# Guoxs/DODT

Hardware: AMD Instinct MI355X
Metric: frame-pairs/sec (whole node) KITTI-shape tau=2 (higher is better)
Workload: dtype f32

## Files before the change

dodt_amd/_lib.py:

```python
import ctypes as C
import os

_HERE = os.path.dirname(os.path.abspath(__file__))
LIB_PATH = os.environ.get('DODT_HIP_LIB') or os.path.join(_HERE, 'lib', 'libdodt_hip.so')

OK, ERR_INVALID, ERR_HIP, ERR_UNSUPPORTED = 0, 1, 2, 3
PTS_VELO_XYZI, PTS_CAM_3XN = 0, 1
EXTRACTOR_VGG_PYR = 0
EXTRACTOR_VGG = 1
EXTRACTOR_SHARED_GPU = 0x100
EXTRACTOR_BF16 = 0x200
EXTRACTOR_SPLIT = 0x400
FC_RELU = 1
FC_BF16 = 2
CONFLICT_RAISE, CONFLICT_NEXT_BEST = 0, 1


class DodtError(RuntimeError):
    pass


class BevParams(C.Structure):
    _fields_ = [
        ('point_format', C.c_int32),
# ... 83 lines not shown
    'dodt_bev_slices': (_i, [_vp, _vp, _i, C.POINTER(BevParams), _pf, _vp]),
    'dodt_bev_status': (_i, [_vp, C.POINTER(_i)]),
    'dodt_bev_support_mask': (_i, [C.POINTER(BevParams), _i, _vp, _i, _i]),
    'dodt_anchor_filter': (_i, [_vp, _vp, _i, _i, _pi32, _i, _i, _pi32, _pi32]),
    'dodt_project_anchors_f64': (_i, [_vp, _vp, _pi32, _i, _pi32,
                                      C.POINTER(_d), C.POINTER(_d), _d, _d,
                                      _pf, _pf, _pf]),
    'dodt_project_anchors_f32': (_i, [_vp, _pf, _i, _pi32, C.POINTER(_f),
                                      C.POINTER(_f), _f, _f, _pf, _pf, _pf]),
    'dodt_img_preprocess': (_i, [_vp, _vp, _i, _i, _i, _i, _i,
                                 C.POINTER(_f), _pf]),
    'dodt_conv_mode': (_i, []),
    'dodt_extractor_create': (_i, [_vp, _i, _i, _i, _i, _i, _i,
                                   C.POINTER(_vp)]),
    'dodt_extractor_destroy': (_i, [_vp]),
    'dodt_extractor_set_layer': (_i, [_vp, C.c_char_p, _vp, _i, _i, _i, _i,
                                      _vp, _vp, _vp]),
    'dodt_extractor_input': (_i, [_vp, C.POINTER(_vp), C.POINTER(C.c_longlong)]),
    'dodt_extractor_forward': (_i, [_vp, _pf, _pf, _pf]),
    'dodt_extractor_forward_padded': (_i, [_vp, _pf, _pf, _pf]),
    'dodt_extractor_set_input': (_i, [_vp, _pf]),
    'dodt_extractor_set_input_support': (_i, [_vp, _vp, _i, _i, C.POINTER(C.c_longlong)]),
    'dodt_extractor_set_frame_tables': (_i, [_vp, _i, C.POINTER(_i)]),
    'dodt_extractor_frame_items': (_i, [_vp, C.POINTER(_i), _i]),
    'dodt_extractor_frame_split': (_i, [_vp, C.POINTER(_i), C.POINTER(_i), _i]),
    'dodt_extractor_store_bytes': (C.c_longlong, [_vp]),
    'dodt_frame_tables_host': (_i, [_vp, _i, _i, _i, _i, _i, _i, _vp, _i, _vp, _vp, C.POINTER(_i)]),
    'dodt_frame_restore_host': (_i, [_vp, _i, _i, _i, _i, _i, _i, _i, _i, _i, _vp, _vp, _vp, _vp]),
    'dodt_frame_lists_host': (_i, [_vp, _i, _i, _i, _i, _i, _i, _vp, _i, _vp, _vp, C.POINTER(_i), _vp, C.POINTER(_i)]),
    'dodt_extractor_read_activation': (_i, [_vp, C.c_char_p, _vp,
                                            C.POINTER(_i), C.POINTER(_i),
                                            C.POINTER(_i)]),
    'dodt_extractor_output_shape': (_i, [_vp, C.POINTER(_i), C.POINTER(_i), C.POINTER(_i)]),
    'dodt_extractor_first_layers_folded': (_i, [_vp]),
    'dodt_extractor_flops': (_d, [_vp]),
    'dodt_extractor_mfma_flops': (_d, [_vp]),
    'dodt_extractor_bytes': (_d, [_vp]),
    'dodt_extractor_layer_count': (_i, [_vp]),
    'dodt_conv_variant_count': (_i, []),
    'dodt_conv_variant_info': (_i, [_i, C.POINTER(ConvVariant)]),
    'dodt_conv_plan_host': (_i, [_i, _i, _i, _i, _i, _i, _i, C.POINTER(ConvLayerPlan), _i, C.POINTER(_i)]),
    'dodt_extractor_layer_plan': (_i, [_vp, C.POINTER(ConvLayerPlan), _i, C.POINTER(_i)]),
    'dodt_extractor_forward_timed': (_i, [_vp, _pf, _pf, _pf, C.POINTER(LayerInfo), _i]),
    'dodt_crop_and_resize': (_i, [_vp, _pf, _i, _i, _i, _pf, _i, _pi32, _i, _i,
                                  _pf]),
    'dodt_crop_and_resize_strided': (_i, [_vp, _pf, _i, _i, _i, _pf, _i, _pi32, _i, _i, _pf,
# ... 90 lines not shown
```

dodt_amd/csrc/conv.hip:

```cpp
#include <cmath>
#include <cstring>

#include <algorithm>
#include <utility>

#include "conv_variants.h"
#include "extractor.h"

using namespace dodt;

const std::vector<KernelVariant>& dodt::variants() {
    static const std::vector<KernelVariant> v = {
        InstSmall<32, 16, 6>::variant(),
        InstSmall<16, 12, 4>::variant(),
        InstSmall<16, 16, 6>::variant(),
        InstSmall<16, 16, 4>::variant(),
        Inst<32, 16, 4, 1, 32, false>::variant(),
        Inst<16, 16, 4, 1, 32, false>::variant(),
        Inst<16, 8, 4, 1, 64, false>::variant(),
        Inst<16, 12, 4, 1, 32, false>::variant(),
        Inst<8, 8, 4, 1, 32, false>::variant(),
        Inst<8, 8, 4, 1, 64, false>::variant(),
        Inst<8, 4, 2, 2, 128, false>::variant(),
        Inst<8, 4, 4, 1, 64, false>::variant(),
// ... 232 lines not shown
        *reinterpret_cast<f32x4*>(out + (size_t)pix * (LPP * 4) + l * 4) = v;
        if (bneck_out) {
            const f32x4 w = *reinterpret_cast<const f32x4*>(bneck_w + l * 4);
            dot = ((v[0] * w[0] + v[1] * w[1]) + v[2] * w[2]) + v[3] * w[3];
        }
    }
    if (bneck_out) {
#pragma unroll
        for (int m = 1; m < LPP; m <<= 1) dot += __shfl_xor(dot, m, 64);
        if (ok && l == 0) bneck_out[pix] = fmaxf(dot * bneck_scale + bneck_shift, 0.0f);
    }
}

int find_layer(dodt_extractor* ex, const char* name) {
    for (size_t i = 0; i < ex->layers.size(); ++i)
        if (ex->layers[i].name == name) return (int)i;
    return -1;
}

void report_launch(const dodt_extractor* ex, const Layer& l, const KernelVariant& v, const ConvArgs& a, int grid_x) {
    if (a.debug & 32) {
        int h[74];
        (void)hipStreamSynchronize(ex->ctx->stream);
        (void)hipMemcpy(h, ex->d_counters + 64 + 32, sizeof(h), hipMemcpyDeviceToHost);
        fprintf(stderr, "[dodt] %s step stamps (cycles): copies | transform | MFMAs | wait copies | barrier | step\n",
                l.name.c_str());
        for (int k = 0; k < 12; ++k)
            fprintf(stderr, "[dodt]   step %2d: %6d %6d %6d %6d %6d   next-top %6d\n", k, h[k * 6 + 1] - h[k * 6],
                    h[k * 6 + 2] - h[k * 6 + 1], h[k * 6 + 3] - h[k * 6 + 2], h[k * 6 + 4] - h[k * 6 + 3],
                    h[k * 6 + 5] - h[k * 6 + 4], k < 11 ? h[(k + 1) * 6] - h[k * 6] : 0);
        if (h[73] != h[72])
            fprintf(stderr, "[dodt]   steps 0..11: %d stamp ticks in %d ticks of the 100 MHz clock (%.0f MHz)\n",
                    h[66] - h[0], h[73] - h[72], 100.0 * (h[66] - h[0]) / (h[73] - h[72]));
    }
    if ((a.debug & 128) && v.dma) {
        std::vector<int> h(4 * grid_x);
        (void)hipStreamSynchronize(ex->ctx->stream);
        (void)hipMemcpy(h.data(), ex->d_counters + 64 + 256, h.size() * sizeof(int), hipMemcpyDeviceToHost);
        int t0 = h[0], s_max = h[0], f_max = h[1], e_min = h[2], e_max = h[2], items[8] = {};
        double first_sum = 0, run_sum = 0;
        for (int b = 0; b < (int)grid_x; ++b) {
            t0 = std::min(t0, h[4 * b]); s_max = std::max(s_max, h[4 * b]);
            f_max = std::max(f_max, h[4 * b + 1]);
            e_min = std::min(e_min, h[4 * b + 2]); e_max = std::max(e_max, h[4 * b + 2]);
            items[std::min(h[4 * b + 3], 7)]++;
            first_sum += (h[4 * b + 1] - h[4 * b]) / 100.0;
            run_sum += (h[4 * b + 2] - h[4 * b + 1]) / 100.0 / std::max(h[4 * b + 3], 1);
        }
        fprintf(stderr, "[dodt] %-16s %4d wgs, %5d items x %d chunks: last start +%.2f us, last first-step +%.2f, first end +%.2f, "
                "last end +%.2f; mean start->first step %.2f us, mean per item %.2f us; wgs by item count:",
                l.name.c_str(), (int)grid_x, a.n_items, a.Cin / 16, (s_max - t0) / 100.0, (f_max - t0) / 100.0,
                (e_min - t0) / 100.0, (e_max - t0) / 100.0, first_sum / grid_x, run_sum / grid_x);
        for (int k = 0; k < 8; ++k) if (items[k]) fprintf(stderr, " %d:%d", k, items[k]);
        int mt[2] = {0, 0};
        (void)hipMemcpy(mt, ex->d_counters + 64 + 250, sizeof(mt), hipMemcpyDeviceToHost);
        fprintf(stderr, "; shader clock of workgroup 1: %.2f GHz\n", (mt[1] - mt[0]) / ((h[4 + 2] - h[4 + 0]) * 10.0));
    }
    if (a.debug & 8) {
        unsigned long long h[2] = {0, 0};
        (void)hipStreamSynchronize(ex->ctx->stream);
        (void)hipMemcpy(h, ex->d_counters + 96, sizeof(h), hipMemcpyDeviceToHost);
        if (h[1])
            fprintf(stderr, "[dodt] %-16s wg0: %.1f us, shader clock %.3f GHz\n", l.name.c_str(),
                    h[1] / 100.0, (double)h[0] / h[1] * 0.1);
    }
}

int launch_grid(const KernelVariant& v, int n_items, int num_cus) {
    static const int bpc_env = getenv("DODT_CONV_BPC") ? atoi(getenv("DODT_CONV_BPC")) : 0;
    static const int small_bpc = getenv("DODT_CONV_SMALL_BPC") ? atoi(getenv("DODT_CONV_SMALL_BPC")) : 3;
    const int vb = v.small_cin ? small_bpc : v.blocks_per_cu;
    const int bpc = (bpc_env > 0 && bpc_env < vb) ? bpc_env : vb;
    return std::min(n_items, num_cus * bpc);
}

int run_launch(const dodt_extractor* ex, const Pass& p, const Layer& l, int which,
               float* override_out, int out_y0, int out_h, float* bneck_out, int pool_dst, const Layer* folded = nullptr) {
    const Launch& ln = which ? l.tail : l.main;
    const size_t li = &l - ex->layers.data();
    const ItemTable& t = p.table[li][which];
    const KernelVariant& v = variants()[folded ? ex->first2_variant : ln.variant];
    const int src_id = folded ? folded->src : l.src;
    const Buffer& src = ex->buf[src_id];
    const Buffer& dst = ex->buf[l.dst];
    ConvArgs a;
    a.in = p.map[src_id];
    a.out = override_out ? override_out : p.map[l.dst];
    a.w = ln.d_w ? ln.d_w : l.main.d_w;
    a.scale = l.d_scale;
    a.shift = l.d_shift;
    a.H = l.H;
    a.W = l.W;
    a.Cin = l.Cin;
    a.Cout = l.Cout;
    a.in_ld = src.C;
    a.in_coff = folded ? folded->src_coff : l.src_coff;
    a.out_ld = dst.C;
    a.out_coff = l.dst_coff;
    a.in_frame_stride = (long long)src.frame_floats();
    a.out_frame_stride = override_out ? (long long)out_h * dst.W * dst.C : (long long)dst.frame_floats();
    a.tiles_x = dodt::ceil_div(l.W, v.TW);
    a.tiles_y = dodt::ceil_div(l.H, v.TH);
    a.relu = 1;
    a.out_y0 = out_y0;
    a.out_nhwc = override_out ? 1 : 0;
    {
        static const int dbg = getenv("DODT_CONV_DEBUG") ? atoi(getenv("DODT_CONV_DEBUG")) : 0;
        a.debug = dbg;
        static const char* stamp_layer = getenv("DODT_CONV_STAMP_LAYER");
        if (stamp_layer && l.name == stamp_layer) a.debug |= 32;
    }
    a.counter = ex->d_counters + 2 * li + which;
    a.counter_base = ex->d_counters + 64;
    a.xcd_counters = variant_xcd_queue(v) ? ex->d_counters + 2048 + 128 * li : nullptr;
    a.items = v.small_cin && t.dense && t.n == a.tiles_x * a.tiles_y * p.frames ? nullptr : t.items;
    a.n_items = t.n;
    if (a.n_items == 0) return DODT_OK;
    a.n_items_dev = t.n_dev;
    a.in_part_stride = (long long)src.frame_floats() * p.frames;
    a.out_part_stride = (long long)dst.frame_floats() * p.frames;
    a.pool_part_stride = pool_dst >= 0 ? (long long)ex->buf[pool_dst].frame_floats() * p.frames : 0;
    a.pool_out = pool_dst >= 0 ? p.map[pool_dst] : nullptr;
    a.pool_frame_stride = pool_dst >= 0 ? (long long)ex->buf[pool_dst].frame_floats() : 0;
    a.bneck_w = bneck_out ? ex->d_bneck_w : nullptr;
    a.bneck_out = bneck_out;
    a.bneck_scale = ex->bneck_scale;
    a.bneck_shift = ex->bneck_shift;
    a.bneck_frame_stride = (long long)out_h * dst.W;
    a.zeros = ex->d_zeros;
    a.first_w = folded ? folded->d_first_w : nullptr;
    a.first_scale = folded ? folded->d_scale : nullptr;
    a.first_shift = folded ? folded->d_shift : nullptr;
    const int grid_x = launch_grid(v, a.n_items, ex->num_cus);
    dim3 grid(grid_x, 1);
    v.launch(a, grid, ex->ctx->stream);
    DODT_LAUNCH_CHECK();
    if (a.debug & (32 | 128 | 8)) report_launch(ex, l, v, a, grid_x);
    return DODT_OK;
}

bool variant_can_pool(const KernelVariant& v) {
    if (v.wino) return true;
    const int rows_per_mt = 32 / v.TW, mt = v.MTB / v.WM;
    return !v.deconv && !v.small_cin && (rows_per_mt >= 2 || mt % 2 == 0) && v.TH % 2 == 0;
}

bool layer_can_pool(const Layer& l) {
    return variant_can_pool(variants()[l.main.variant]) &&
           (l.tail.n_items == 0 || variant_can_pool(variants()[l.tail.variant]));
}

int run_layer(const dodt_extractor* ex, const Pass& p, const Layer& l, float* override_out, int out_y0, int out_h,
              float* bneck_out = nullptr, int pool_dst = -1, const Layer* folded = nullptr) {
    if (p.timed && folded) {
        DODT_HIP_CHECK(hipEventRecord(folded->ev0, ex->ctx->stream));
        DODT_HIP_CHECK(hipEventRecord(folded->ev1, ex->ctx->stream));
// ... 109 lines not shown
    const Buffer& s = ex->buf[src];
    const Buffer& d = ex->buf[dst];
    const int planes = d.C / 8;
    const long long total = (long long)p.frames * planes * d.H * d.W * 2;
    hipLaunchKernelGGL(maxpool2x2_kernel, dim3((unsigned)((total + 255) / 256)), dim3(256), 0,
                       ex->ctx->stream, p.map[src], s.H, s.W, planes, (long long)s.frame_floats(),
                       p.map[dst], p.frames);
    DODT_LAUNCH_CHECK();
    return DODT_OK;
}

int forward(dodt_extractor* ex, const float* d_in, const float* d_x0, float* d_feat_out, float* d_bottleneck_out,
            bool timed);

}

int dodt::fused_pool_buffer(const Layer& l) {
    static const bool no_fuse = getenv("DODT_CONV_NO_POOL_FUSE") != nullptr;
    return no_fuse || !layer_can_pool(l) ? -1 : l.pool;
}

bool dodt::bneck_fused(const Layer& last) {
    return variants()[last.main.variant].BN == 32 && (last.tail.n_items == 0 || variants()[last.tail.variant].BN == 32);
}

int dodt::run_layers(const dodt_extractor* ex, const Pass& p, float* d_feat_out, float* d_bottleneck_out) {
    hipStream_t s = ex->ctx->stream;
    int rc;
    const std::vector<Layer>& ls = ex->layers;
    if (ex->bf16)
        for (int id : {CONV1_2, CONV2_2, CONV3_3})
            DODT_REQUIRE(fused_pool_buffer(ls[id]) >= 0, "bf16 extractor: layer %s cannot pool in its epilogue",
                         ls[id].name.c_str());
    for (int id = ex->first2_variant >= 0 ? CONV1_2 : CONV1_1; id <= CONV4_3; ++id) {
        const Layer& l = ls[id];
        const Layer* folded = id == CONV1_2 && ex->first2_variant >= 0 ? &ls[CONV1_1] : nullptr;
        const int pool_dst = folded ? l.pool : fused_pool_buffer(l);
        if ((rc = run_layer(ex, p, l, nullptr, 0, 0, nullptr, pool_dst, folded))) return rc;
        if (l.pool >= 0 && pool_dst < 0 && (rc = run_pool(ex, p, l.dst, l.pool))) return rc;
    }
    if (ex->kind == DODT_EXTRACTOR_VGG) {
        const Buffer& c4 = ex->buf[C4C];
        const long long n_pix = (long long)p.frames * ex->out_h * ex->out_w;
        constexpr int kLpp = 64;
        hipLaunchKernelGGL(upsample_bilinear_cb8_kernel<kLpp>,
                           dim3((unsigned)((n_pix * kLpp + 255) / 256)), dim3(256), 0, s, p.map[C4C],
// ... 92 lines not shown
    for (Layer& l : plan.layers) {
        plan_layer(l, batch, num_cus, !shared_gpu, l.main.h_items, l.tail.h_items);
        l.main.n_items = (int)l.main.h_items.size();
        l.tail.n_items = (int)l.tail.h_items.size();
    }
    {
        static const bool first2 = !(getenv("DODT_CONV_BF16_FIRST2") && atoi(getenv("DODT_CONV_BF16_FIRST2")) == 0);
        const Layer& c11 = plan.layers[CONV1_1];
        const Layer& c12 = plan.layers[CONV1_2];
        const auto& vs = variants();
        if (first2 && bf16 && plan.parts == 1 && vs[c12.variant].stream_nch == 2 && c12.tail.n_items == 0 &&
            c11.Cout == 32 && c11.src_coff == 0 && (W * c11.Cin * 4) % 16 == 0 &&
            variant_can_pool(vs[c12.variant]))
            for (size_t i = 0; i < vs.size() && plan.first2_variant < 0; ++i)
                if (vs[i].first2 == c11.Cin && vs[i].TH == vs[c12.variant].TH && vs[i].TW == vs[c12.variant].TW &&
                    vs[i].lds_bytes <= (getenv("DODT_CONV_BF16_STREAM_LDS") ? atoi(getenv("DODT_CONV_BF16_STREAM_LDS")) * 1024 : 1 << 30))
                    plan.first2_variant = (int)i;
    }
    return DODT_OK;
}

namespace {

void report_layer(const std::vector<Layer>& layers, int first2_variant, int num_cus, size_t i, dodt_conv_layer_plan* o) {
    const Layer& l = layers[i];
    const bool folding = first2_variant >= 0;
    memset(o, 0, sizeof(*o));
    snprintf(o->name, sizeof(o->name), "%s", l.name.c_str());
    o->h = l.H; o->w = l.W; o->cin = l.Cin; o->cout = l.Cout;
    o->variant[0] = l.main.variant;
    o->variant[1] = l.tail.n_items > 0 ? l.tail.variant : -1;
    o->items[0] = l.main.n_items;
    o->items[1] = l.tail.n_items;
    if (folding && i == CONV1_1) {
        o->variant[0] = -1;
        o->items[0] = 0;
        o->folded = 1;
    }
    if (folding && i == CONV1_2) o->variant[0] = first2_variant;
    for (int j = 0; j < 2; ++j)
        o->grid[j] = o->variant[j] >= 0 ? launch_grid(variants()[o->variant[j]], o->items[j], num_cus) : 0;
    o->pool_fused = l.pool >= 0 && ((folding && i == CONV1_2) || fused_pool_buffer(l) >= 0);
    o->bneck_fused = i == FUSION1 && bneck_fused(l);
}

int report_plan(const std::vector<Layer>& layers, int first2_variant, int num_cus, dodt_conv_layer_plan* out, int n_out,
                int* n_layers) {
    if (n_layers) *n_layers = (int)layers.size();
    if (!out) return DODT_OK;
    DODT_REQUIRE(n_out >= (int)layers.size(), "conv plan: room for %d layers, the net has %d", n_out, (int)layers.size());
    for (size_t i = 0; i < layers.size(); ++i) report_layer(layers, first2_variant, num_cus, i, out + i);
    return DODT_OK;
}

}

extern "C" {

int dodt_conv_plan_host(int kind, int in_h, int in_w, int in_c, int pad_top, int batch, int num_cus,
                        dodt_conv_layer_plan* out, int n_out, int* n_layers) {
    ConvPlan plan;
    const int rc = plan_convs(kind, in_h, in_w, in_c, pad_top, batch, num_cus, plan);
    return rc ? rc : report_plan(plan.layers, plan.first2_variant, num_cus, out, n_out, n_layers);
}

int dodt_extractor_layer_plan(const dodt_extractor* ex, dodt_conv_layer_plan* out, int n_out, int* n_layers) {
    DODT_REQUIRE(ex, "dodt_extractor_layer_plan: extractor is NULL");
    return report_plan(ex->layers, ex->first2_variant, ex->num_cus, out, n_out, n_layers);
}

int dodt_conv_variant_count(void) { return (int)variants().size(); }

int dodt_conv_variant_info(int i, dodt_conv_variant* out) {
    DODT_REQUIRE(out && i >= 0 && i < (int)variants().size(), "dodt_conv_variant_info: bad argument");
    const KernelVariant& v = variants()[i];
    memset(out, 0, sizeof(*out));
    out->tw = v.TW; out->th = v.TH; out->bn = v.BN; out->ck = v.CK;
    out->blocks_per_cu = v.blocks_per_cu;
    out->flags = (v.deconv ? DODT_VARIANT_DECONV : 0) | (v.small_cin ? DODT_VARIANT_SMALL_CIN : 0) |
                 (v.tail_only ? DODT_VARIANT_TAIL_ONLY : 0) | (v.bf16 ? DODT_VARIANT_BF16 : 0) |
                 (v.parts == 2 ? DODT_VARIANT_SPLIT : 0) | (v.wino ? DODT_VARIANT_WINO : 0) |
                 (v.wino && v.wino_m == 4 ? DODT_VARIANT_WINO43 : 0) | (v.dma ? DODT_VARIANT_DMA : 0) |
                 (v.deconv_dma ? DODT_VARIANT_DECONV_DMA : 0) | (v.first2 ? DODT_VARIANT_FIRST2 : 0) |
                 (v.stream_nch ? DODT_VARIANT_STREAM : 0) | (variant_xcd_queue(v) ? DODT_VARIANT_XCD_QUEUE : 0) |
                 (variant_can_pool(v) ? DODT_VARIANT_CAN_POOL : 0);
    out->lds_bytes = v.lds_bytes;
    snprintf(out->kernel, sizeof(out->kernel), "%s", kernel_name(v));
    return DODT_OK;
}

int dodt_extractor_create(dodt_ctx* ctx, int kind, int in_h, int in_w, int in_c, int pad_top,
// ... 30 lines not shown
    if (!plain) { setb(F3, H4, W4, 64); setb(F2, H2, W2, 32); setb(F1, H, W, 32); }
    if (plain) {
        ex->out_h = (int)((double)in_h / 8.0 * 4.0);
        ex->out_w = (int)((double)in_w / 8.0 * 4.0);
        ex->out_c = 256;
    } else {
        ex->out_h = in_h; ex->out_w = in_w; ex->out_c = 32;
    }
    for (int i = 0; i < NBUF; ++i) {
        ex->buf[i].bf16 = bf16 && i != X0 && i != F1;
        ex->buf[i].parts = ex->buf[i].bf16 ? ex->parts : 1;
    }
    for (int i = 0; i < NBUF; ++i) {
        if (i == F1 || ex->buf[i].H == 0) continue;
        const size_t bytes = ex->buf[i].frame_floats() * batch * ex->buf[i].parts * sizeof(float);
        hipError_t e = hipMalloc(&ex->buf[i].ptr, bytes);
        if (e != hipSuccess) {
            dodt::set_error("dodt_extractor_create: hipMalloc(%zu) failed: %s", bytes,
                            hipGetErrorString(e));
            dodt_extractor_destroy(ex);
            return DODT_ERR_HIP;
        }
    }
    DODT_HIP_CHECK(hipMalloc(&ex->d_counters, 4096 * sizeof(int)));
    DODT_HIP_CHECK(hipMemsetAsync(ex->d_counters, 0, 4096 * sizeof(int), ctx->stream));
    DODT_HIP_CHECK(hipMalloc(&ex->d_zeros, 256));
    DODT_HIP_CHECK(hipMemsetAsync(ex->d_zeros, 0, 256, ctx->stream));
    DODT_HIP_CHECK(hipMemsetAsync(ex->buf[X0].ptr, 0,
                                  ex->buf[X0].frame_floats() * batch * sizeof(float), ctx->stream));

    ex->layers = std::move(plan.layers);
    ex->first2_variant = plan.first2_variant;
    for (Layer& l : ex->layers) {
        for (Launch* ln : {&l.main, &l.tail}) {
            if (ln->h_items.empty()) continue;
            DODT_HIP_CHECK(hipMalloc(&ln->d_items, ln->h_items.size() * sizeof(int4)));
            DODT_HIP_CHECK(hipMemcpyAsync(ln->d_items, ln->h_items.data(), ln->h_items.size() * sizeof(int4),
                                          hipMemcpyHostToDevice, ctx->stream));
        }
    }
    DODT_HIP_CHECK(hipStreamSynchronize(ctx->stream));
    if (getenv("DODT_DEBUG_PLAN")) {
        if (ex->first2_variant >= 0) fprintf(stderr, "[dodt] conv1_1 runs folded into conv1_2's launch\n");
        for (const Layer& l : ex->layers) {
            const KernelVariant& v = variants()[l.variant];
            fprintf(stderr, "[dodt] %-16s %4dx%-4d %3d->%-3d TW%d TH%d BN%d CK%d lds %d items %d",
                    l.name.c_str(), l.H, l.W, l.Cin, l.Cout, v.TW, v.TH, v.BN, v.CK, v.lds_bytes,
                    l.main.n_items);
// ... 126 lines not shown
    DODT_REQUIRE(ex && d_feat_out, "dodt_extractor_forward: NULL argument");
    for (const Layer& l : ex->layers)
        DODT_REQUIRE(l.loaded, "dodt_extractor_forward: weights of layer %s not set",
                     l.name.c_str());
    DODT_REQUIRE(!d_bottleneck_out || ex->bneck_loaded,
                 "dodt_extractor_forward: bottleneck weights not set");
    hipStream_t s = ex->ctx->stream;
    Pass p;
    for (int i = 0; i < NBUF; ++i) p.map[i] = ex->buf[i].ptr;
    if (d_x0) p.map[X0] = const_cast<float*>(d_x0);
    p.frames = ex->batch;
    p.timed = timed;
    const Buffer& x0 = ex->buf[X0];
    float* own_in = p.map[X0] + (size_t)ex->pad_top * x0.W * x0.C;
    if (d_in && d_in != own_in) {
        const long long n4 = (long long)ex->in_h * ex->in_w * ex->in_c / 4;
        DODT_REQUIRE(((long long)ex->in_h * ex->in_w * ex->in_c) % 4 == 0, "input not float4-sized");
        hipLaunchKernelGGL(copy_rows_kernel, dim3((unsigned)((n4 * ex->batch + 255) / 256)),
                           dim3(256), 0, s, reinterpret_cast<const float4*>(d_in),
                           reinterpret_cast<float4*>(own_in), n4, n4,
                           (long long)x0.frame_floats() / 4, ex->batch);
        DODT_LAUNCH_CHECK();
    }
    DODT_HIP_CHECK(hipMemsetAsync(ex->d_counters, 0, 4096 * sizeof(int), s));
    const bool skip = ex->skip_on && ex->primed;
    const int known = find_pair(ex, d_feat_out, d_bottleneck_out);
    const bool last_skip = skip && known >= 0;
    choose_tables(ex, skip, last_skip, p);
    const int slot = known >= 0 ? ex->pairs[known].slot : slot_for_new_pair(ex);
    int rc;
    if (ex->frame_on && (rc = begin_frame_forward(ex, p, slot, last_skip, d_feat_out, d_bottleneck_out))) return rc;
    if ((rc = run_layers(ex, p, d_feat_out, d_bottleneck_out))) return rc;
    if (ex->skip_on) {
        ex->primed = true;
        if (known < 0) add_pair(ex, d_feat_out, d_bottleneck_out, slot);
    }
    return DODT_OK;
}

}

extern "C" {

int dodt_extractor_output_shape(const dodt_extractor* ex, int* h, int* w, int* c) {
    DODT_REQUIRE(ex, "dodt_extractor_output_shape: NULL argument");
    if (h) *h = ex->out_h;
    if (w) *w = ex->out_w;
    if (c) *c = ex->out_c;
    return DODT_OK;
}

// ... 138 lines not shown
```

dodt_amd/csrc/conv_bf16_dma.h:

```cpp
#pragma once
#include <hip/hip_runtime.h>

#include <type_traits>

#include "conv_kernels.h"
#include "wino_kernels.h"

namespace dodt {

struct StreamTile { int frame, ty0, tx0; };
template <int MODE, int MT, int NT = 1, int NTI = 0>
__device__ __forceinline__ void stream_epilogue(const ConvArgs& a, const float* p_scale, const float* p_shift, const float* p_bw,
                                                f32x16 (&acc_all)[MT * NT], const StreamTile cur, int c0, int wave, int li, int lh,
                                                bool stamp, int* stamps, float* s_tile = nullptr) {
    auto acc = [&](int mt) -> f32x16& { return acc_all[mt * NT + NTI]; };
    const float floor_v = a.relu ? 0.0f : -3.0e38f;
    {
        f32x4 sc[4], sh[4];
#pragma unroll
        for (int g = 0; g < 4; ++g) {
            const int c = group_channel<true>(g, lh);
            sc[g] = *reinterpret_cast<const f32x4*>(p_scale + c);
            sh[g] = *reinterpret_cast<const f32x4*>(p_shift + c);
        }
// ... 633 lines not shown
    const int lane = tid & 63;
    const int wave = __builtin_amdgcn_readfirstlane(tid >> 6);
    const int producer_wave = 3 - (int)((blockIdx.x / ((gridDim.x + 1) / 2)) & 1);
    const bool producer = wave == producer_wave;
    const int cw = wave < producer_wave ? wave : wave - 1;
    const int li = lane & 31, lh = lane >> 5;

    const int tiles_per_frame = a.tiles_x * a.tiles_y;
    auto decode = [&](int it) {
        it = __builtin_amdgcn_readfirstlane(it);
        const int f = it / tiles_per_frame, r = it - f * tiles_per_frame;
        const int ty = r / a.tiles_x;
        return StreamTile{f, ty * Cfg::TH, (r - ty * a.tiles_x) * Cfg::TW};
    };
    const bool grouped = a.xcd_counters != nullptr;
    const int vx = grouped ? (int)(blockIdx.x & 7) : 0;
    const int q_lo = grouped ? vx * (a.n_items / 8) + min(vx, a.n_items % 8) : 0;
    const int q_hi = grouped ? q_lo + a.n_items / 8 + (vx < a.n_items % 8 ? 1 : 0) : a.n_items;
    const int q_blocks = grouped ? ((int)gridDim.x - vx + 7) / 8 : (int)gridDim.x;
    const int q_first = q_lo + q_blocks;
    int* const q_counter = grouped ? a.xcd_counters + 16 * vx : a.counter;
    auto ticket_item = [&](int t) { return q_first + t < q_hi ? q_first + t : a.n_items; };
    const int k_first = q_lo + (grouped ? (int)(blockIdx.x >> 3) : (int)blockIdx.x);
    if (k_first >= q_hi) return;
    if (tid < 128)
        s_par[tid] = tid < 32 ? a.scale[tid] : tid < 64 ? a.shift[tid - 32]
                   : tid < 96 ? a.first_scale[tid - 64] : a.first_shift[tid - 96];
    auto queue_at = [&](int n) { return __builtin_amdgcn_readfirstlane(s_q[n & 15]); };
    int ticket = 0;
    if (tid == 0) {
        s_q[0] = k_first;
        const int t = atomicAdd(q_counter, S + 1);
#pragma unroll
        for (int i = 0; i < S; ++i) s_q[1 + i] = ticket_item(t + i);
        ticket = t + S;
    }
    const unsigned lds0 = (unsigned)(size_t)(__attribute__((address_space(3))) void*)smem;

    if (producer) {
        int p_off[KC];
        i32x4_t in_rsrc;
        const int row_bytes = a.W * Cfg::kPixBytes;
        auto setup = [&](int item) {
            if (item >= a.n_items) {
                in_rsrc = make_rsrc(a.in, 0u);
                return;
// ... 235 lines not shown
```

dodt_amd/csrc/conv_kernels.h:

```cpp
#pragma once
#include <hip/hip_runtime.h>

namespace dodt {

typedef float f32x16 __attribute__((ext_vector_type(16)));
typedef float f32x4 __attribute__((ext_vector_type(4)));

struct ConvArgs {
    const float* in;
    float* out;
    const float* w;
    const float* scale;
    const float* shift;
    int H, W;
    int Cin, Cout;
    int in_ld, in_coff, out_ld, out_coff;
    long long in_frame_stride, out_frame_stride;
    int tiles_x, tiles_y;
    const int4* items;
    int n_items;
    int relu;
    int out_y0;
    int out_nhwc;
    int* counter;
    int* counter_base;
    float* pool_out;
    long long pool_frame_stride;
    const float* bneck_w;
    float* bneck_out;
    float bneck_scale, bneck_shift;
    long long bneck_frame_stride;
    long long in_part_stride, out_part_stride, pool_part_stride;
    const float* zeros;
    int debug;
    int* xcd_counters;
    const float* first_w;
    const float* first_scale;
    const float* first_shift;
    const int* n_items_dev;
};

constexpr int kCK = 8;
constexpr int kPixStride = 12;

template <int TW, int MTB, int WM, int WN, int BN, bool DECONV, int PARTS = 1>
struct ConvCfg {
    static constexpr int kRowsPerMT = 32 / TW;
    static constexpr int TH = MTB * kRowsPerMT;
    static constexpr int PH = DECONV ? TH + 1 : TH + 2;
    static constexpr int PW = DECONV ? TW + 1 : TW + 2;
    static constexpr int MT = MTB / WM;
    static constexpr int NT = BN / 32 / WN;
    static constexpr int kPitchTarget = TW == 16 ? 0 : TW == 8 ? 8 : TW == 4 ? 4 : -1;
    static constexpr int pitch_for(int pw) {
        int pr = pw * kPixStride;
        if (kPitchTarget >= 0)
            while ((pr / 4) % 16 != kPitchTarget) pr += 4;
        return pr;
    }
    static constexpr int kMinWaves0 = PARTS == 2 ? 1 : 2;
    static constexpr int resident_for(int pr) {
        const int lds = 2 * PARTS * (PH * pr + 9 * kCK * BN) * 4 + 16;
        const int r = (160 * 1024) / lds;
// ... 626 lines not shown
        const int frame = item.x, ty0 = item.z, tx0 = item.w;
        const float* in = a.in + (size_t)frame * a.in_frame_stride;
#pragma unroll
        for (int i = 0; i < NIT; ++i) {
            const int t = tid + 256 * i;
            const int cg = t % CG, p = t / CG;
            const int py = p / PW, px = p - py * PW;
            const int gy = ty0 - 1 + py, gx = tx0 - 1 + px;
#pragma unroll
            for (int k = 0; k < VEC; ++k) v[i][k] = 0.0f;
            if (t < ITEMS && gy >= 0 && gy < a.H && gx >= 0 && gx < a.W) {
                const float* src = in + ((size_t)gy * a.W + gx) * a.in_ld + a.in_coff + cg * VEC;
                if constexpr (VEC == 4) {
                    const float4 q = *reinterpret_cast<const float4*>(src);
                    v[i][0] = q.x; v[i][1] = q.y; v[i][2] = q.z; v[i][3] = q.w;
                } else {
                    const float2 q = *reinterpret_cast<const float2*>(src);
                    v[i][0] = q.x; v[i][1] = q.y;
                }
            }
        }
    };
    int bid = blockIdx.x;
    if (bid >= n_items) return;
    {
        float4 wv[NW];
        const float4* wsrc = reinterpret_cast<const float4*>(a.w);
#pragma unroll
        for (int i = 0; i < NW; ++i) {
            const int t = tid + 256 * i;
            wv[i] = t < Cfg::kWFloats / 4 ? wsrc[t] : float4{0.f, 0.f, 0.f, 0.f};
        }
        load_patch(bid);
#pragma unroll
        for (int i = 0; i < NW; ++i) {
            const int t = tid + 256 * i;
            if (t < Cfg::kWFloats / 4) reinterpret_cast<float4*>(sW)[t] = wv[i];
        }
    }
    const int x_base = lh * PS + (li / TW) * PW + (li % TW) + wm * MT * Cfg::kRowsPerMT * PW;
    const int w_base = lh * BN + li;
    const long long plane = (long long)a.H * a.W * 8;
    int buf = 0;
    for (; bid < n_items; bid += gridDim.x) {
        float* sP = smem + buf * Cfg::kPatchFloats;
#pragma unroll
// ... 44 lines not shown
```

dodt_amd/csrc/conv_skip.hip:

```cpp
#include <algorithm>
#include <cstring>

#include "conv_variants.h"
#include "extractor.h"

using namespace dodt;
using dodt::ft::RestoreTable;
using dodt::ft::RestorePlan;

namespace {

struct Support {
    int h = 0, w = 0;
    std::vector<uint8_t> m;
    Support() = default;
    Support(int h_, int w_) : h(h_), w(w_), m((size_t)h_ * w_, 0) {}
    uint8_t& at(int y, int x) { return m[(size_t)y * w + x]; }
    uint8_t at(int y, int x) const { return m[(size_t)y * w + x]; }
};

Support dilate(const Support& a, int r) {
    Support t(a.h, a.w), o(a.h, a.w);
    for (int y = 0; y < a.h; ++y)
        for (int x = 0; x < a.w; ++x)
// ... 185 lines not shown
        ex->store_bytes = total + px * (ex->out_c + 1) * sizeof(float);
    }
    Temps temps;
    Pass p;
    p.frames = 1;
    for (int i = 0; i < NBUF; ++i) p.map[i] = ex->store[i];
    const size_t in_bytes = ex->buf[X0].frame_floats() * sizeof(float);
    DODT_HIP_CHECK(temps.alloc((void**)&p.map[X0], in_bytes));
    DODT_HIP_CHECK(hipMemsetAsync(p.map[X0], 0, in_bytes, s));
    for (size_t li = 0; li < ex->layers.size(); ++li) {
        const Layer& l = ex->layers[li];
        const std::vector<int4>& mi = l.main.h_items;
        const int n0 = (int)(std::find_if(mi.begin(), mi.end(), [](const int4& it) { return it.x != 0; }) - mi.begin());
        p.table[li][0] = {l.main.d_items, n0, nullptr, true};
        std::vector<int4> first;
        for (const int4& it : l.tail.h_items)
            if (it.x == 0) first.push_back(it);
        if (first.empty()) continue;
        int4* d = nullptr;
        DODT_HIP_CHECK(temps.alloc((void**)&d, first.size() * sizeof(int4)));
        DODT_HIP_CHECK(hipMemcpy(d, first.data(), first.size() * sizeof(int4), hipMemcpyHostToDevice));
        p.table[li][1] = {d, (int)first.size(), nullptr, false};
    }
    DODT_HIP_CHECK(hipMemsetAsync(ex->d_counters, 0, 4096 * sizeof(int), s));
    const int rc = run_layers(ex, p, ex->store_feat, ex->bneck_loaded ? ex->store_bneck : nullptr);
    DODT_HIP_CHECK(hipStreamSynchronize(s));
    if (rc) return rc;
    RestorePlan pl;
    for (size_t li = 0; li < ex->layers.size(); ++li) {
        const Layer& l = ex->layers[li];
        const int pool_dst = fused_pool_buffer(l);
        int j = 0;
        for (const Launch* ln : {&l.main, &l.tail}) {
            const ft::Table& ft = ex->frame_plan.t[2 * li + j];
            RestoreTable& t = pl.t[2 * li + j++];
            if (!ft.items) continue;
            const Buffer& dst = ex->buf[l.dst];
            t.list = ft.restore;
            t.count = ft.rcount;
            t.dst = dst.ptr;
            t.src = ex->store[l.dst];
            t.frame_stride = (long long)dst.frame_floats();
            t.H = dst.H; t.W = dst.W;
            t.ch0 = l.dst_coff;
            t.bn = variants()[ln->variant].BN;
            t.f = ft.f; t.th = ft.th; t.tw = ft.tw;
            if (pool_dst >= 0) {
// ... 60 lines not shown
    for (size_t li = 0; li < ex->layers.size(); ++li) {
        const Layer& l = ex->layers[li];
        const bool on = li == (size_t)FUSION1 ? last_skip : skip;
        const Tables kind = !on ? Tables::Full : ex->frame_on ? Tables::PerFrame : Tables::Static;
        ex->ran[li].kind = kind;
        int j = 0;
        for (const Launch* ln : {&l.main, &l.tail}) {
            ItemTable& t = p.table[li][j];
            if (kind == Tables::Full || ln->n_skip < 0) t = {ln->d_items, ln->n_items, nullptr, true};
            else if (kind == Tables::PerFrame && ln->d_run) t = {ln->d_run, ln->n_skip, ln->d_count, false};
            else t = {ln->d_skip, ln->n_skip, nullptr, false};
            ex->ran[li].n[j++] = t.n;
        }
    }
    ex->restoring = ex->frame_on && skip;
}

int begin_frame_forward(dodt_extractor* ex, const Pass& p, int slot, bool last_skip, float* d_feat_out,
                        float* d_bottleneck_out) {
    hipStream_t s = ex->ctx->stream;
    int rc;
    if (ex->restoring && !ex->store_valid) {
        if ((rc = take_store(ex))) return rc;
        DODT_HIP_CHECK(hipMemsetAsync(ex->d_counters, 0, 4096 * sizeof(int), s));
    }
    if ((rc = build_frame_tables(ex, p, slot))) return rc;
    if (ex->restoring) {
        hipLaunchKernelGGL(frame_restore_kernel, dim3((unsigned)(4 * ex->ctx->num_cus)), dim3(256), 0, s,
                           ex->d_restore_plan, d_feat_out, d_bottleneck_out, last_skip ? 1 : 0);
        DODT_LAUNCH_CHECK();
    }
    return DODT_OK;
}

WorkShare::WorkShare(const dodt_extractor* ex) : have(false) {
    if (!ex->frame_on) return;
    if (hipStreamSynchronize(ex->ctx->stream) != hipSuccess) return;
    have = hipMemcpy(counts, ex->d_frame_counts, sizeof(counts), hipMemcpyDeviceToHost) == hipSuccess;
}

double WorkShare::restore_bytes(const dodt_extractor* ex, const Layer& l) const {
    const size_t li = &l - ex->layers.data();
    const bool pooled = fused_pool_buffer(l) >= 0;
    const bool bneck = &l == &ex->layers.back() && ex->bneck_loaded && bneck_fused(l);
    double b = 0.0;
    int j = 0;
    for (const Launch* ln : {&l.main, &l.tail}) {
// ... 121 lines not shown
            DODT_HIP_CHECK(alloc(t.n, (void**)&t.now));
            if (li == (size_t)FUSION1) {
                for (int k = 0; k < kOutPairs; ++k) DODT_HIP_CHECK(alloc(t.n, (void**)&ex->out_prev[k][jj]));
            } else {
                DODT_HIP_CHECK(alloc(t.n, (void**)&t.prev));
            }
            DODT_HIP_CHECK(alloc(t.n * sizeof(int4), (void**)&t.run));
            t.count = ex->d_frame_counts + 2 * li + jj;
            DODT_HIP_CHECK(alloc(t.n * sizeof(int4), (void**)&t.restore));
            t.rcount = ex->d_frame_counts + ft::kTables + 2 * li + jj;
            ln->d_run = t.run;
            ln->d_count = t.count;
        }
    }
    DODT_HIP_CHECK(alloc(sizeof(ft::Plan), (void**)&ex->d_frame_plan));
    DODT_HIP_CHECK(hipMemcpy(ex->d_frame_plan, &pl, sizeof(ft::Plan), hipMemcpyHostToDevice));
    ex->primed = false;
    forget_pairs(ex);
    ex->frame_on = true;
    if (enabled) *enabled = 1;
    return DODT_OK;
}

int dodt_extractor_frame_items(dodt_extractor* ex, int* items, int n) {
    DODT_REQUIRE(ex && items && n >= (int)ex->layers.size(),
                 "dodt_extractor_frame_items: items must hold dodt_extractor_layer_count() entries");
    const WorkShare share(ex);
    for (size_t i = 0; i < ex->layers.size(); ++i)
        items[i] = share.per_frame(ex, i) ? share.items(i, 0) + share.items(i, 1) + share.restored(ex, i, 0) +
                                                share.restored(ex, i, 1)
                                          : -1;
    return DODT_OK;
}

int dodt_extractor_frame_split(dodt_extractor* ex, int* computed, int* restored, int n) {
    DODT_REQUIRE(ex && computed && restored && n >= (int)ex->layers.size(),
                 "dodt_extractor_frame_split: computed and restored must hold dodt_extractor_layer_count() entries");
    const WorkShare share(ex);
    for (size_t i = 0; i < ex->layers.size(); ++i) {
        const bool pf = share.per_frame(ex, i);
        computed[i] = pf ? share.items(i, 0) + share.items(i, 1) : -1;
        restored[i] = pf ? share.restored(ex, i, 0) + share.restored(ex, i, 1) : -1;
    }
    return DODT_OK;
}

// ... 98 lines not shown
```

dodt_amd/csrc/extractor.h:

```cpp
#pragma once
#include <string>
#include <vector>

#include "common.h"
#include "frame_tables.h"

namespace dodt {

struct KernelVariant;

struct Buffer {
    int H = 0, W = 0, C = 0;
    float* ptr = nullptr;
    bool bf16 = false;
    int parts = 1;
    size_t frame_floats() const { return (size_t)H * W * C / (bf16 ? 2 : 1); }
};

struct Launch {
    int variant = -1;
    int n_items = 0;
    int4* d_items = nullptr;
    float* d_w = nullptr;
    std::vector<int4> h_items;
// ... 25 lines not shown

enum LayerId {
    CONV1_1, CONV1_2, CONV2_1, CONV2_2, CONV3_1, CONV3_2, CONV3_3, CONV4_1, CONV4_2, CONV4_3,
    UPCONV3, FUSION3, UPCONV2, FUSION2, UPCONV1, FUSION1, NLAYERS
};
static_assert(NLAYERS == ft::kLayers, "the per-frame builder walks the pyramid net's layers");
static_assert(ft::transposed(UPCONV3) && ft::transposed(UPCONV2) && ft::transposed(UPCONV1) && !ft::transposed(FUSION1) &&
                  !ft::transposed(CONV4_3), "the per-frame builder's transposed convs are the net's");

enum class Tables { Full, Static, PerFrame };

struct ItemTable {
    const int4* items = nullptr;
    int n = 0;
    const int* n_dev = nullptr;
    bool dense = false;
};

struct Pass {
    float* map[NBUF] = {};
    int frames = 0;
    bool timed = false;
    ItemTable table[NLAYERS][2];
};

struct OutPair {
    const float* feat = nullptr;
    const float* bneck = nullptr;
    int slot = 0;
};
constexpr int kOutPairs = 8;

struct ConvPlan {
    int kind = DODT_EXTRACTOR_VGG_PYR;
    bool bf16 = false;
    int parts = 1;
    int H = 0, W = 0;
    std::vector<Layer> layers;
    int first2_variant = -1;
};

}

struct dodt_extractor {
    dodt_ctx* ctx = nullptr;
    int in_h = 0, in_w = 0, in_c = 0, pad_top = 0, batch = 0;
    int kind = DODT_EXTRACTOR_VGG_PYR;
    int out_h = 0, out_w = 0, out_c = 32;
    bool bf16 = false;
    int parts = 1;
    int H = 0, W = 0;
    int num_cus = 0;
    dodt::Buffer buf[dodt::NBUF];
    std::vector<dodt::Layer> layers;
    float* d_bneck_w = nullptr;
    int* d_counters = nullptr;
    float* d_zeros = nullptr;
    float bneck_scale = 1.0f, bneck_shift = 0.0f;
    bool bneck_loaded = false;
    double flops = 0.0;
    int first2_variant = -1;
    float* own_x0 = nullptr;
    bool skip_on = false;
    bool primed = false;
    dodt::OutPair pairs[dodt::kOutPairs];
    int n_pairs = 0;
    struct Ran {
        dodt::Tables kind = dodt::Tables::Full;
        int n[2] = {0, 0};
    } ran[dodt::NLAYERS];
    bool restoring = false;
    bool frame_on = false;
    dodt::ft::Plan frame_plan;
    dodt::ft::Plan* d_frame_plan = nullptr;
    uint32_t* d_frame_bits = nullptr;
    int* d_frame_counts = nullptr;
    std::vector<void*> frame_allocs;
    uint8_t* out_prev[dodt::kOutPairs][2] = {};
    float* store[dodt::NBUF] = {};
    float* store_feat = nullptr;
    float* store_bneck = nullptr;
    dodt::ft::RestorePlan* d_restore_plan = nullptr;
    bool store_valid = false;
    size_t store_bytes = 0;
};

namespace dodt {

const std::vector<KernelVariant>& variants();
int fused_pool_buffer(const Layer& l);
bool bneck_fused(const Layer& last);
int plan_convs(int kind, int in_h, int in_w, int in_c, int pad_top, int batch, int num_cus, ConvPlan& plan);
int run_layers(const dodt_extractor* ex, const Pass& p, float* d_feat_out, float* d_bottleneck_out);

struct WeightTile {
    int BN, CK;
    bool bf16, small_cin;
    int parts;
};
std::vector<float> block_deconv_dma(const WeightTile& v, const Layer& l, const float* w, int cin, int cout);
std::vector<float> block_wino43(const WeightTile& v, const Layer& l, const float* w, int cin, int cout);
std::vector<float> block_wino22(const WeightTile& v, const Layer& l, const float* w, int cin, int cout);
std::vector<float> block_direct(const WeightTile& v, const Layer& l, const float* w, int cin, int cout);
std::vector<uint16_t> pack_first2(const Layer& l, const float* w, int cin, int cout);
template <class T>
int upload(T** d, const std::vector<T>& h, hipStream_t s) {
    if (!*d) DODT_HIP_CHECK(hipMalloc(d, h.size() * sizeof(T)));
    DODT_HIP_CHECK(hipMemcpyAsync(*d, h.data(), h.size() * sizeof(T), hipMemcpyHostToDevice, s));
    DODT_HIP_CHECK(hipStreamSynchronize(s));
    return DODT_OK;
}

void free_frame_tables(dodt_extractor* ex);
int find_pair(const dodt_extractor* ex, const float* feat, const float* bneck);
int slot_for_new_pair(const dodt_extractor* ex);
// ... 25 lines not shown
```

include/dodt_hip.h:

```cpp
#ifndef DODT_HIP_H
#define DODT_HIP_H

#include <stddef.h>
#include <stdint.h>

#ifdef __cplusplus
extern "C" {
#endif

#define DODT_OK 0
#define DODT_ERR_INVALID 1
#define DODT_ERR_HIP 2
#define DODT_ERR_UNSUPPORTED 3

typedef struct dodt_ctx dodt_ctx;

int dodt_version(void);
const char* dodt_last_error(void);
int dodt_ctx_create(int device_id, dodt_ctx** out);
int dodt_ctx_create_high_priority(int device_id, dodt_ctx** out);
int dodt_ctx_create_on_stream(int device_id, void* hip_stream, dodt_ctx** out);
int dodt_ctx_destroy(dodt_ctx* ctx);
int dodt_ctx_set_plan_cus(dodt_ctx* ctx, int n);
int dodt_ctx_sync(dodt_ctx* ctx);
// ... 66 lines not shown
typedef struct dodt_extractor dodt_extractor;
#define DODT_EXTRACTOR_VGG_PYR 0
#define DODT_EXTRACTOR_VGG 1
#define DODT_EXTRACTOR_SHARED_GPU 0x100
#define DODT_EXTRACTOR_BF16 0x200
#define DODT_EXTRACTOR_SPLIT 0x400
#define DODT_CONV_MODE_DEFAULT 2
int dodt_conv_mode(void);
int dodt_extractor_create(dodt_ctx* ctx, int kind, int in_h, int in_w, int in_c,
                          int pad_top, int batch, dodt_extractor** out);
int dodt_extractor_destroy(dodt_extractor* ex);
int dodt_extractor_set_layer(dodt_extractor* ex, const char* name, const float* w,
                             int kh, int kw, int c_a, int c_b, const float* beta,
                             const float* mean, const float* var);
int dodt_extractor_input(dodt_extractor* ex, float** d_ptr, long long* frame_stride_floats);
int dodt_extractor_forward(dodt_extractor* ex, const float* d_in, float* d_feat_out,
                           float* d_bottleneck_out);
int dodt_extractor_forward_padded(dodt_extractor* ex, const float* d_x0, float* d_feat_out,
                                  float* d_bottleneck_out);
int dodt_extractor_set_input(dodt_extractor* ex, const float* d_x0);
int dodt_extractor_set_input_support(dodt_extractor* ex, const uint8_t* mask, int rows, int cols,
                                     long long* skipped_items);
int dodt_extractor_set_frame_tables(dodt_extractor* ex, int on, int* enabled);
int dodt_extractor_frame_items(dodt_extractor* ex, int* items, int n);
int dodt_extractor_frame_split(dodt_extractor* ex, int* computed, int* restored, int n);
long long dodt_extractor_store_bytes(const dodt_extractor* ex);
int dodt_frame_tables_host(const uint8_t* masks, int frames, int rows, int cols, int layer, int th, int tw,
                           const int* items, int n_items, const uint8_t* prev, int* run, int* n_run);
int dodt_frame_lists_host(const uint8_t* masks, int frames, int rows, int cols, int layer, int th, int tw,
                          const int* items, int n_items, const uint8_t* prev, int* run, int* n_run, int* restore,
                          int* n_restore);
int dodt_frame_restore_host(const int* item, int f, int th, int tw, int bn, int ch0, int rows, int cols, int channels,
                            int pad_top, float* dst, const float* src, float* dst2, const float* src2);
int dodt_extractor_output_shape(const dodt_extractor* ex, int* h, int* w, int* c);
int dodt_extractor_first_layers_folded(const dodt_extractor* ex);
int dodt_extractor_read_activation(dodt_extractor* ex, const char* name, float* dst,
                                   int* h, int* w, int* c);
double dodt_extractor_flops(const dodt_extractor* ex);
double dodt_extractor_mfma_flops(const dodt_extractor* ex);
double dodt_extractor_bytes(const dodt_extractor* ex);
typedef struct dodt_layer_info {
    char name[32];
    char kernel[48];
    int32_t launches;
    int32_t items;
    double flops_direct;
// ... 204 lines not shown
```

Measured before the change: 422.5.

## Double-buffer conv counters cleared in-kernel and add a workgroup slot budget

The per-forward memset of the 4096-word work-queue counter buffer is replaced by two counter banks. The first conv kernel of each pass zeroes the other bank while running, and a memset is kept only when that layer has no items. This removes one memset launch from the stream per forward. It also adds an API that caps each conv launch's grid at a workgroup budget (default 0, meaning no cap), so several extractors can share the GPU. The cost is a little extra work in the first kernel, plus a dependence on the bank alternation staying correct across skip and restore paths.

```diff
diff --git a/dodt_amd/_lib.py b/dodt_amd/_lib.py
--- a/dodt_amd/_lib.py
+++ b/dodt_amd/_lib.py
@@ -129,6 +129,8 @@
     'dodt_extractor_set_input': (_i, [_vp, _pf]),
     'dodt_extractor_set_input_support': (_i, [_vp, _vp, _i, _i, C.POINTER(C.c_longlong)]),
     'dodt_extractor_set_frame_tables': (_i, [_vp, _i, C.POINTER(_i)]),
+    'dodt_extractor_set_slot_budget': (_i, [_vp, _i]),
+    'dodt_conv_grid_host': (_i, [_i, _i, _i, _i, C.POINTER(_i)]),
     'dodt_extractor_frame_items': (_i, [_vp, C.POINTER(_i), _i]),
     'dodt_extractor_frame_split': (_i, [_vp, C.POINTER(_i), C.POINTER(_i), _i]),
     'dodt_extractor_store_bytes': (C.c_longlong, [_vp]),
diff --git a/dodt_amd/csrc/conv.hip b/dodt_amd/csrc/conv.hip
--- a/dodt_amd/csrc/conv.hip
+++ b/dodt_amd/csrc/conv.hip
@@ -278,7 +278,7 @@
     if (a.debug & 32) {
         int h[74];
         (void)hipStreamSynchronize(ex->ctx->stream);
-        (void)hipMemcpy(h, ex->d_counters + 64 + 32, sizeof(h), hipMemcpyDeviceToHost);
+        (void)hipMemcpy(h, a.counter_base + 32, sizeof(h), hipMemcpyDeviceToHost);
         fprintf(stderr, "[dodt] %s step stamps (cycles): copies | transform | MFMAs | wait copies | barrier | step\n",
                 l.name.c_str());
         for (int k = 0; k < 12; ++k)
@@ -292,7 +292,7 @@
     if ((a.debug & 128) && v.dma) {
         std::vector<int> h(4 * grid_x);
         (void)hipStreamSynchronize(ex->ctx->stream);
-        (void)hipMemcpy(h.data(), ex->d_counters + 64 + 256, h.size() * sizeof(int), hipMemcpyDeviceToHost);
+        (void)hipMemcpy(h.data(), a.counter_base + 256, h.size() * sizeof(int), hipMemcpyDeviceToHost);
         int t0 = h[0], s_max = h[0], f_max = h[1], e_min = h[2], e_max = h[2], items[8] = {};
         double first_sum = 0, run_sum = 0;
         for (int b = 0; b < (int)grid_x; ++b) {
@@ -309,25 +309,25 @@
                 (e_min - t0) / 100.0, (e_max - t0) / 100.0, first_sum / grid_x, run_sum / grid_x);
         for (int k = 0; k < 8; ++k) if (items[k]) fprintf(stderr, " %d:%d", k, items[k]);
         int mt[2] = {0, 0};
-        (void)hipMemcpy(mt, ex->d_counters + 64 + 250, sizeof(mt), hipMemcpyDeviceToHost);
+        (void)hipMemcpy(mt, a.counter_base + 250, sizeof(mt), hipMemcpyDeviceToHost);
         fprintf(stderr, "; shader clock of workgroup 1: %.2f GHz\n", (mt[1] - mt[0]) / ((h[4 + 2] - h[4 + 0]) * 10.0));
     }
     if (a.debug & 8) {
         unsigned long long h[2] = {0, 0};
         (void)hipStreamSynchronize(ex->ctx->stream);
-        (void)hipMemcpy(h, ex->d_counters + 96, sizeof(h), hipMemcpyDeviceToHost);
+        (void)hipMemcpy(h, a.counter_base + 32, sizeof(h), hipMemcpyDeviceToHost);
         if (h[1])
             fprintf(stderr, "[dodt] %-16s wg0: %.1f us, shader clock %.3f GHz\n", l.name.c_str(),
                     h[1] / 100.0, (double)h[0] / h[1] * 0.1);
     }
 }
 
-int launch_grid(const KernelVariant& v, int n_items, int num_cus) {
+int launch_grid(const KernelVariant& v, int n_items, int num_cus, int budget) {
     static const int bpc_env = getenv("DODT_CONV_BPC") ? atoi(getenv("DODT_CONV_BPC")) : 0;
     static const int small_bpc = getenv("DODT_CONV_SMALL_BPC") ? atoi(getenv("DODT_CONV_SMALL_BPC")) : 3;
     const int vb = v.small_cin ? small_bpc : v.blocks_per_cu;
     const int bpc = (bpc_env > 0 && bpc_env < vb) ? bpc_env : vb;
-    return std::min(n_items, num_cus * bpc);
+    return dodt::capped_grid(n_items, num_cus * bpc, budget);
 }
 
 int run_launch(const dodt_extractor* ex, const Pass& p, const Layer& l, int which,
@@ -366,9 +366,12 @@
         static const char* stamp_layer = getenv("DODT_CONV_STAMP_LAYER");
         if (stamp_layer && l.name == stamp_layer) a.debug |= 32;
     }
-    a.counter = ex->d_counters + 2 * li + which;
-    a.counter_base = ex->d_counters + 64;
-    a.xcd_counters = variant_xcd_queue(v) ? ex->d_counters + 2048 + 128 * li : nullptr;
+    a.counter = p.counters + 2 * li + which;
+    a.counter_base = p.counters + 64;
+    a.xcd_counters = variant_xcd_queue(v) ? p.counters + 2048 + 128 * li : nullptr;
+    a.clear_bank = which == 0 && (folded || li == (size_t)CONV1_1) ? p.clear : nullptr;
+    DODT_REQUIRE(!a.clear_bank || v.small_cin || v.first2, "layer %s: its kernel does not zero the counter bank",
+                 l.name.c_str());
     a.items = v.small_cin && t.dense && t.n == a.tiles_x * a.tiles_y * p.frames ? nullptr : t.items;
     a.n_items = t.n;
     if (a.n_items == 0) return DODT_OK;
@@ -387,7 +390,7 @@
     a.first_w = folded ? folded->d_first_w : nullptr;
     a.first_scale = folded ? folded->d_scale : nullptr;
     a.first_shift = folded ? folded->d_shift : nullptr;
-    const int grid_x = launch_grid(v, a.n_items, ex->num_cus);
+    const int grid_x = launch_grid(v, a.n_items, ex->num_cus, ex->slot_cap);
     dim3 grid(grid_x, 1);
     v.launch(a, grid, ex->ctx->stream);
     DODT_LAUNCH_CHECK();
@@ -543,6 +546,12 @@
 
 bool dodt::bneck_fused(const Layer& last) {
     return variants()[last.main.variant].BN == 32 && (last.tail.n_items == 0 || variants()[last.tail.variant].BN == 32);
+}
+
+void dodt::take_counter_bank(dodt_extractor* ex, Pass& p) {
+    p.counters = ex->d_counters + ex->bank * kCounterWords;
+    ex->bank ^= 1;
+    p.clear = ex->d_counters + ex->bank * kCounterWords;
 }
 
 int dodt::run_layers(const dodt_extractor* ex, const Pass& p, float* d_feat_out, float* d_bottleneck_out) {
@@ -681,7 +690,8 @@
 
 namespace {
 
-void report_layer(const std::vector<Layer>& layers, int first2_variant, int num_cus, size_t i, dodt_conv_layer_plan* o) {
+void report_layer(const std::vector<Layer>& layers, int first2_variant, int num_cus, int budget, size_t i,
+                  dodt_conv_layer_plan* o) {
     const Layer& l = layers[i];
     const bool folding = first2_variant >= 0;
     memset(o, 0, sizeof(*o));
@@ -698,17 +708,17 @@
     }
     if (folding && i == CONV1_2) o->variant[0] = first2_variant;
     for (int j = 0; j < 2; ++j)
-        o->grid[j] = o->variant[j] >= 0 ? launch_grid(variants()[o->variant[j]], o->items[j], num_cus) : 0;
+        o->grid[j] = o->variant[j] >= 0 ? launch_grid(variants()[o->variant[j]], o->items[j], num_cus, budget) : 0;
     o->pool_fused = l.pool >= 0 && ((folding && i == CONV1_2) || fused_pool_buffer(l) >= 0);
     o->bneck_fused = i == FUSION1 && bneck_fused(l);
 }
 
-int report_plan(const std::vector<Layer>& layers, int first2_variant, int num_cus, dodt_conv_layer_plan* out, int n_out,
+int report_plan(const std::vector<Layer>& layers, int first2_variant, int num_cus, int budget, dodt_conv_layer_plan* out, int n_out,
                 int* n_layers) {
     if (n_layers) *n_layers = (int)layers.size();
     if (!out) return DODT_OK;
     DODT_REQUIRE(n_out >= (int)layers.size(), "conv plan: room for %d layers, the net has %d", n_out, (int)layers.size());
-    for (size_t i = 0; i < layers.size(); ++i) report_layer(layers, first2_variant, num_cus, i, out + i);
+    for (size_t i = 0; i < layers.size(); ++i) report_layer(layers, first2_variant, num_cus, budget, i, out + i);
     return DODT_OK;
 }
 
@@ -720,12 +730,19 @@
                         dodt_conv_layer_plan* out, int n_out, int* n_layers) {
     ConvPlan plan;
     const int rc = plan_convs(kind, in_h, in_w, in_c, pad_top, batch, num_cus, plan);
-    return rc ? rc : report_plan(plan.layers, plan.first2_variant, num_cus, out, n_out, n_layers);
+    return rc ? rc : report_plan(plan.layers, plan.first2_variant, num_cus, 0, out, n_out, n_layers);
 }
 
 int dodt_extractor_layer_plan(const dodt_extractor* ex, dodt_conv_layer_plan* out, int n_out, int* n_layers) {
     DODT_REQUIRE(ex, "dodt_extractor_layer_plan: extractor is NULL");
-    return report_plan(ex->layers, ex->first2_variant, ex->num_cus, out, n_out, n_layers);
+    return report_plan(ex->layers, ex->first2_variant, ex->num_cus, ex->slot_cap, out, n_out, n_layers);
+}
+
+int dodt_conv_grid_host(int variant, int n_items, int num_cus, int budget, int* grid) {
+    DODT_REQUIRE(grid && variant >= 0 && variant < (int)variants().size() && n_items >= 0 && num_cus >= 1 && budget >= 0,
+                 "dodt_conv_grid_host: bad argument");
+    *grid = launch_grid(variants()[variant], n_items, num_cus, budget);
+    return DODT_OK;
 }
 
 int dodt_conv_variant_count(void) { return (int)variants().size(); }
@@ -802,8 +819,8 @@
             return DODT_ERR_HIP;
         }
     }
-    DODT_HIP_CHECK(hipMalloc(&ex->d_counters, 4096 * sizeof(int)));
-    DODT_HIP_CHECK(hipMemsetAsync(ex->d_counters, 0, 4096 * sizeof(int), ctx->stream));
+    DODT_HIP_CHECK(hipMalloc(&ex->d_counters, 2 * kCounterWords * sizeof(int)));
+    DODT_HIP_CHECK(hipMemsetAsync(ex->d_counters, 0, 2 * kCounterWords * sizeof(int), ctx->stream));
     DODT_HIP_CHECK(hipMalloc(&ex->d_zeros, 256));
     DODT_HIP_CHECK(hipMemsetAsync(ex->d_zeros, 0, 256, ctx->stream));
     DODT_HIP_CHECK(hipMemsetAsync(ex->buf[X0].ptr, 0,
@@ -976,11 +993,13 @@
                            (long long)x0.frame_floats() / 4, ex->batch);
         DODT_LAUNCH_CHECK();
     }
-    DODT_HIP_CHECK(hipMemsetAsync(ex->d_counters, 0, 4096 * sizeof(int), s));
+    take_counter_bank(ex, p);
     const bool skip = ex->skip_on && ex->primed;
     const int known = find_pair(ex, d_feat_out, d_bottleneck_out);
     const bool last_skip = skip && known >= 0;
     choose_tables(ex, skip, last_skip, p);
+    if (p.table[ex->first2_variant >= 0 ? CONV1_2 : CONV1_1][0].n == 0)
+        DODT_HIP_CHECK(hipMemsetAsync(p.clear, 0, kCounterWords * sizeof(int), s));
     const int slot = known >= 0 ? ex->pairs[known].slot : slot_for_new_pair(ex);
     int rc;
     if (ex->frame_on && (rc = begin_frame_forward(ex, p, slot, last_skip, d_feat_out, d_bottleneck_out))) return rc;
diff --git a/dodt_amd/csrc/conv_bf16_dma.h b/dodt_amd/csrc/conv_bf16_dma.h
--- a/dodt_amd/csrc/conv_bf16_dma.h
+++ b/dodt_amd/csrc/conv_bf16_dma.h
@@ -679,6 +679,7 @@
     int* const q_counter = grouped ? a.xcd_counters + 16 * vx : a.counter;
     auto ticket_item = [&](int t) { return q_first + t < q_hi ? q_first + t : a.n_items; };
     const int k_first = q_lo + (grouped ? (int)(blockIdx.x >> 3) : (int)blockIdx.x);
+    clear_counter_bank(a);
     if (k_first >= q_hi) return;
     if (tid < 128)
         s_par[tid] = tid < 32 ? a.scale[tid] : tid < 64 ? a.shift[tid - 32]
diff --git a/dodt_amd/csrc/conv_kernels.h b/dodt_amd/csrc/conv_kernels.h
--- a/dodt_amd/csrc/conv_kernels.h
+++ b/dodt_amd/csrc/conv_kernels.h
@@ -38,7 +38,15 @@
     const float* first_scale;
     const float* first_shift;
     const int* n_items_dev;
+    int* clear_bank;
 };
+
+constexpr int kCounterWords = 4096;
+
+__device__ __forceinline__ void clear_counter_bank(const ConvArgs& a) {
+    if (!a.clear_bank) return;
+    for (int i = blockIdx.x * blockDim.x + threadIdx.x; i < kCounterWords; i += gridDim.x * blockDim.x) a.clear_bank[i] = 0;
+}
 
 constexpr int kCK = 8;
 constexpr int kPixStride = 12;
@@ -711,6 +719,7 @@
         }
     };
     int bid = blockIdx.x;
+    clear_counter_bank(a);
     if (bid >= n_items) return;
     {
         float4 wv[NW];
diff --git a/dodt_amd/csrc/conv_skip.hip b/dodt_amd/csrc/conv_skip.hip
--- a/dodt_amd/csrc/conv_skip.hip
+++ b/dodt_amd/csrc/conv_skip.hip
@@ -231,7 +231,8 @@
         DODT_HIP_CHECK(hipMemcpy(d, first.data(), first.size() * sizeof(int4), hipMemcpyHostToDevice));
         p.table[li][1] = {d, (int)first.size(), nullptr, false};
     }
-    DODT_HIP_CHECK(hipMemsetAsync(ex->d_counters, 0, 4096 * sizeof(int), s));
+    DODT_HIP_CHECK(hipMemsetAsync(ex->d_counters, 0, 2 * kCounterWords * sizeof(int), s));
+    p.counters = ex->d_counters;
     const int rc = run_layers(ex, p, ex->store_feat, ex->bneck_loaded ? ex->store_bneck : nullptr);
     DODT_HIP_CHECK(hipStreamSynchronize(s));
     if (rc) return rc;
@@ -338,7 +339,7 @@
     int rc;
     if (ex->restoring && !ex->store_valid) {
         if ((rc = take_store(ex))) return rc;
-        DODT_HIP_CHECK(hipMemsetAsync(ex->d_counters, 0, 4096 * sizeof(int), s));
+        DODT_HIP_CHECK(hipMemsetAsync(ex->d_counters, 0, 2 * kCounterWords * sizeof(int), s));
     }
     if ((rc = build_frame_tables(ex, p, slot))) return rc;
     if (ex->restoring) {
@@ -506,6 +507,12 @@
     return DODT_OK;
 }
 
+int dodt_extractor_set_slot_budget(dodt_extractor* ex, int workgroups) {
+    DODT_REQUIRE(ex && workgroups >= 0, "dodt_extractor_set_slot_budget: NULL extractor or a negative budget");
+    ex->slot_cap = workgroups;
+    return DODT_OK;
+}
+
 int dodt_extractor_frame_items(dodt_extractor* ex, int* items, int n) {
     DODT_REQUIRE(ex && items && n >= (int)ex->layers.size(),
                  "dodt_extractor_frame_items: items must hold dodt_extractor_layer_count() entries");
diff --git a/dodt_amd/csrc/extractor.h b/dodt_amd/csrc/extractor.h
--- a/dodt_amd/csrc/extractor.h
+++ b/dodt_amd/csrc/extractor.h
@@ -1,4 +1,5 @@
 #pragma once
+#include <algorithm>
 #include <string>
 #include <vector>
 
@@ -71,7 +72,14 @@
     int frames = 0;
     bool timed = false;
     ItemTable table[NLAYERS][2];
-};
+    int* counters = nullptr;
+    int* clear = nullptr;
+};
+
+inline int capped_grid(int n_items, int resident, int budget) {
+    const int g = std::min(n_items, resident);
+    return budget > 0 ? std::min(g, std::max(budget, 8)) : g;
+}
 
 struct OutPair {
     const float* feat = nullptr;
@@ -104,6 +112,8 @@
     std::vector<dodt::Layer> layers;
     float* d_bneck_w = nullptr;
     int* d_counters = nullptr;
+    int bank = 0;
+    int slot_cap = 0;
     float* d_zeros = nullptr;
     float bneck_scale = 1.0f, bneck_shift = 0.0f;
     bool bneck_loaded = false;
@@ -140,6 +150,7 @@
 int fused_pool_buffer(const Layer& l);
 bool bneck_fused(const Layer& last);
 int plan_convs(int kind, int in_h, int in_w, int in_c, int pad_top, int batch, int num_cus, ConvPlan& plan);
+void take_counter_bank(dodt_extractor* ex, Pass& p);
 int run_layers(const dodt_extractor* ex, const Pass& p, float* d_feat_out, float* d_bottleneck_out);
 
 struct WeightTile {
diff --git a/include/dodt_hip.h b/include/dodt_hip.h
--- a/include/dodt_hip.h
+++ b/include/dodt_hip.h
@@ -112,6 +112,8 @@
 int dodt_extractor_set_input_support(dodt_extractor* ex, const uint8_t* mask, int rows, int cols,
                                      long long* skipped_items);
 int dodt_extractor_set_frame_tables(dodt_extractor* ex, int on, int* enabled);
+int dodt_extractor_set_slot_budget(dodt_extractor* ex, int workgroups);
+int dodt_conv_grid_host(int variant, int n_items, int num_cus, int budget, int* grid);
 int dodt_extractor_frame_items(dodt_extractor* ex, int* items, int n);
 int dodt_extractor_frame_split(dodt_extractor* ex, int* computed, int* restored, int n);
 long long dodt_extractor_store_bytes(const dodt_extractor* ex);
```

New measurement: 418.9. No clear change (-0.8%).
